# calclavia/tal-asrd

Measured on AMD Instinct MI355X. Metric: audio frames/sec (16 kHz, 10 ms hop) end-to-end log-mel -> TDS encoder -> diarization head, higher is better.
Workload: dtype f32 (dense layers: 3 x f16 MFMA hi/lo split, f32 accumulate)

## Files before the change

tal_asrd_amd/csrc/api.hip:

```cpp
#include <string.h>

#include <atomic>

#include "common.h"

namespace tal {

static thread_local char g_err[512] = "";

void set_error(const char* fmt, ...) {
    va_list ap;
    va_start(ap, fmt);
    vsnprintf(g_err, sizeof(g_err), fmt, ap);
    va_end(ap);
}

static const char* const g_opt_names[OPT_COUNT] = {
    "tds_exact_f32", "tds_fp32_activations", "gconv_fuse_split", "gconv_c1_generic", "head_no_astationary", "gemm_global_loads",
    "gemm_no_splitk4", "gemm_no_glds", "gemm_no_splitk_tail", "gemm_no_w64", "logmel_no_fold", "decode_no_small", "decode_small_rows", "gemm_no_row_split", "gemm_no_n96", "gemm_s64_below", "gconv_short_below", "gconv_no_shift18", "gconv_grid_xyz", "gemm_w64_stagger", "gemm_s64_order", "decode_wide_gemm", "gemm_s64_rows", "decode_persist", "decode_persist_wgs", "logmel_mfma", "gru_unfused", "decode_no_fold", "gconv_c1_fuse", "decode_fold_rows", "gconv_long_tt", "logmel_general"};
static std::atomic<int> g_opt[OPT_COUNT] = {{0}, {0}, {0}, {0}, {0}, {0}, {0}, {0}, {0}, {0}, {0}, {0}, {256}, {0}, {0}, {2}, {4}, {0}, {0}, {0}, {0}, {0}, {0}, {0}, {32}, {0}, {0}, {0}, {0}, {64}, {0}, {0}};
int opt(Option o) { return g_opt[o].load(std::memory_order_relaxed); }

int device_cus() {
    static std::atomic<int> table[64];
    int dev = 0;
    if (hipGetDevice(&dev) != hipSuccess || dev < 0 || dev >= 64) dev = 0;
    int cus = table[dev].load(std::memory_order_relaxed);
    if (!cus) {
        hipDeviceProp_t p;
        if (hipGetDeviceProperties(&p, dev) == hipSuccess) cus = p.multiProcessorCount;
        if (cus <= 0) cus = 256;
        table[dev].store(cus, std::memory_order_relaxed);
    }
    return cus;
}

static const int PROF_MAX = 8192;
static std::atomic<bool> g_prof_on{false};
static std::atomic<int> g_prof_n{0};
static hipEvent_t g_prof_ev[PROF_MAX][2];
static std::atomic<int> g_prof_have[PROF_MAX];
static int g_prof_cls[PROF_MAX];
static double g_prof_work[PROF_MAX];

ProfScope::ProfScope(int cls, double work, hipStream_t stream) : slot(-1), s(stream) {
    if (!g_prof_on.load(std::memory_order_relaxed)) return;
    const int mine = g_prof_n.fetch_add(1, std::memory_order_relaxed);
    if (mine >= PROF_MAX) return;
    g_prof_cls[mine] = -1;
    if (!g_prof_have[mine].load(std::memory_order_acquire)) {
        if (hipEventCreate(&g_prof_ev[mine][0]) != hipSuccess || hipEventCreate(&g_prof_ev[mine][1]) != hipSuccess)
            return;
        g_prof_have[mine].store(1, std::memory_order_release);
    }
    slot = mine;
    g_prof_cls[slot] = cls;
    g_prof_work[slot] = work;
    (void)hipEventRecord(g_prof_ev[slot][0], s);
}
ProfScope::~ProfScope() {
    if (slot >= 0) (void)hipEventRecord(g_prof_ev[slot][1], s);
}

__global__ __launch_bounds__(256) void argmax_rows_kernel(const float* __restrict__ x, int64_t M, int N,
                                                         int32_t* __restrict__ ids) {
    const int lane = threadIdx.x & 63;
    const int64_t row = (int64_t)blockIdx.x * 4 + (threadIdx.x >> 6);
    if (row >= M) return;
    const float* xr = x + row * N;
    float best = -INFINITY;
    int bi = 0x7fffffff;
    for (int i = lane; i < N; i += 64) {
        const float v = xr[i];
// ... 701 lines not shown
```

tal_asrd_amd/csrc/common.h:

```cpp
#pragma once
#include <hip/hip_runtime.h>
#include <stdint.h>
#include <stdio.h>
#include <stdarg.h>
#include <stdlib.h>

#include "../../include/tal_asrd.h"

namespace tal {

void set_error(const char* fmt, ...);

#define TAL_CHECK_ARG(cond, ...)                 \
    do {                                         \
        if (!(cond)) {                           \
            tal::set_error(__VA_ARGS__);         \
            return TAL_EINVAL;                   \
        }                                        \
    } while (0)

#define TAL_CHECK_LAUNCH(what)                                                        \
    do {                                                                              \
        hipError_t e__ = hipGetLastError();                                           \
        if (e__ != hipSuccess) {                                                      \
// ... 35 lines not shown
__device__ __forceinline__ void reset_ticket(unsigned* word) {
    __hip_atomic_store(word, 0u, __ATOMIC_RELAXED, __HIP_MEMORY_SCOPE_AGENT);
}

__device__ __forceinline__ float amax4(float a, const f32x4& v) {
    return fmaxf(fmaxf(a, fmaxf(fabsf(v.x), fabsf(v.y))), fmaxf(fabsf(v.z), fabsf(v.w)));
}
__device__ __forceinline__ void note_range(float amax, int* flag) {
    if (flag && amax > 65504.f) atomicOr(flag, 1);
}

typedef float f32x2p __attribute__((ext_vector_type(2)));
typedef _Float16 f16x2p __attribute__((ext_vector_type(2)));
__device__ __forceinline__ void split_f16x3_pair(float a, float b, f16x2p& hi, f16x2p& lo) {
    const f32x2p x = {a, b};
    hi = __builtin_convertvector(x, f16x2p);
    const f32x2p hf = __builtin_convertvector(hi, f32x2p);
    lo = __builtin_convertvector((x - hf) * 2048.f, f16x2p);
}

enum Option {
    OPT_TDS_EXACT_F32 = 0,
    OPT_TDS_FP32_ACTIVATIONS,
    OPT_GCONV_FUSE_SPLIT,
    OPT_GCONV_C1_GENERIC,
    OPT_HEAD_NO_ASTATIONARY,
    OPT_GEMM_GLOBAL_LOADS,
    OPT_GEMM_NO_SPLITK4,
    OPT_GEMM_NO_GLDS,
    OPT_GEMM_NO_SPLITK_TAIL,
    OPT_GEMM_NO_W64,
    OPT_LOGMEL_NO_FOLD,
    OPT_DECODE_NO_SMALL,
    OPT_DECODE_SMALL_ROWS,
    OPT_GEMM_NO_ROW_SPLIT,
    OPT_GEMM_NO_N96,
    OPT_GEMM_S64_BELOW,
    OPT_GCONV_SHORT_BELOW,
    OPT_GCONV_NO_SHIFT18,
    OPT_GCONV_GRID_XYZ,
    OPT_GEMM_W64_STAGGER,
    OPT_GEMM_S64_ORDER,
    OPT_DECODE_WIDE_GEMM,
    OPT_GEMM_S64_ROWS,
    OPT_DECODE_PERSIST,
    OPT_DECODE_PERSIST_WGS,
    OPT_LOGMEL_MFMA,
    OPT_GRU_UNFUSED,
    OPT_DECODE_NO_FOLD,
    OPT_GCONV_C1_FUSE,
    OPT_DECODE_FOLD_ROWS,
    OPT_GCONV_LONG_TT,
    OPT_LOGMEL_GENERAL,
    OPT_COUNT
};
int opt(Option o);
int device_cus();

__device__ __forceinline__ unsigned xcd_logical_block(unsigned nb, unsigned bid) {
    const unsigned xcd = bid & 7u, q = nb >> 3, r = nb & 7u;
    return (xcd < r ? xcd * (q + 1) : r * (q + 1) + (xcd - r) * q) + (bid >> 3);
}

__device__ __forceinline__ int wave_id() { return __builtin_amdgcn_readfirstlane((int)(threadIdx.x >> 6)); }

enum ProfClass { PROF_GEMM = 0, PROF_GCONV_RES = 1, PROF_GCONV_S2 = 2, PROF_LOGMEL = 3, PROF_OTHER = 4, PROF_NCLASS = 5 };
struct ProfScope {
    int slot;
    hipStream_t s;
    ProfScope(int cls, double work, hipStream_t stream);
    ~ProfScope();
};

struct GemmArgs {
    const float* A;
    const float* W;
    const float* bias;
    const float* res;
    float* Y;
    int64_t M;
    int N, K;
    int64_t lda, ldw, ldy, ldres;
    int nb2;
    int64_t a_s1, a_s2, w_s1, w_s2, y_s1, y_s2, r_s1, r_s2, bias_s2;
    float alpha;
    int scale_cols;
    int tiles_n;
    unsigned tiles_n_magic;
    float* part_val;
    int32_t* part_idx;
    int part_ld;
    int tile_base, split, tail_tiles;
    float* splitk_ws;
    size_t splitk_ws_bytes;
    int f16x3, out_split;
    int res_split;
    int* range_flag;
    int stagger_ticks, stagger_blocks;
    int n_major, tiles_m;
    unsigned tiles_m_magic;
};
int launch_gemm(GemmArgs g, int mode, int nbatch, hipStream_t s);
void launch_gemm_w64(const GemmArgs& g, int mode, bool splitk, dim3 grid, hipStream_t s);
bool gemm_s64_ok(const GemmArgs& g, int mode);
void launch_gemm_s64(GemmArgs g, int mode, hipStream_t s);
int gemm_mode4_partials(int64_t M, int N);
// ... 120 lines not shown
```

tal_asrd_amd/csrc/gconv.hip:

```cpp
#include "common.h"

namespace tal {

constexpr int KS = 21;

template <int CIG, int COG, int STRIDE, int GB, int TT, bool RESID>
__global__ __launch_bounds__(256) void gconv_kernel(const float* __restrict__ x, const float* __restrict__ wp,
                                                   const float* __restrict__ bias, float alpha,
                                                   float* __restrict__ y, int64_t T_in, int64_t T_out, int C_in,
                                                   int C_out) {
    constexpr int PAD = RESID ? KS / 2 : 0;
    constexpr int TIN = (TT - 1) * STRIDE + KS;
    constexpr int TINP = TIN | 1;
    constexpr int WPG = GB >= 4 ? 1 : 4 / GB;
    constexpr int TW = TT / WPG;
    constexpr int R = TW / 64;
    static_assert(TW % 64 == 0 && R >= 1, "time tile per wave must be a multiple of 64");
    constexpr int CH = GB * CIG;
    extern __shared__ __attribute__((aligned(16))) float xs[];

    const int b = blockIdx.z;
    const int g0 = blockIdx.y * GB;
    const int64_t t0 = (int64_t)blockIdx.x * TT;
    const int tid = threadIdx.x;
// ... 337 lines not shown
    }
    return false;
}

template <int P>
__device__ __forceinline__ f16x8 gconv_frag(const _Float16* p, const _Float16* p2) {
    if (P % 8 == 0) return *reinterpret_cast<const f16x8*>(p);
#ifdef GC_MERGED_READS
    if (P % 4 == 0) return *reinterpret_cast<const f16x8a8*>(p);
#endif
    if (P % 4 == 0) {
        typedef _Float16 f16x4a8 __attribute__((ext_vector_type(4), aligned(8)));
        const f16x4a8 a = *reinterpret_cast<const f16x4a8*>(p), b = *reinterpret_cast<const f16x4a8*>(p2);
        return f16x8{a[0], a[1], a[2], a[3], b[0], b[1], b[2], b[3]};
    }
    return *reinterpret_cast<const f16x8u*>(p);
}

#ifdef GC_TIMELINE
__device__ unsigned long long g_gc_timeline[8 * 4 * 4096];
#define GC_STAMP(i)                                                                                   \
    do {                                                                                              \
        if ((threadIdx.x & 63) == 0 && blockIdx.x < 4096)                                             \
            g_gc_timeline[((i) * 4 + (threadIdx.x >> 6)) * 4096 + blockIdx.x] = wall_clock64();       \
    } while (0)
#else
#define GC_STAMP(i)
#endif

#define GC_BLOCK_INDEX(n_tt, n_gb)                                                           \
    int b, g0;                                                                               \
    int64_t t0;                                                                              \
    if (n_tt > 0) {                                                                          \
        const unsigned L = xcd_logical_block(gridDim.x, blockIdx.x);                         \
        const unsigned gbi = L % (unsigned)n_gb, rest = L / (unsigned)n_gb;                  \
        g0 = (int)gbi * GB;                                                                  \
        t0 = (int64_t)(rest % (unsigned)n_tt) * TT;                                          \
        b = (int)(rest / (unsigned)n_tt);                                                    \
    } else {                                                                                 \
        b = blockIdx.z;                                                                      \
        g0 = blockIdx.y * GB;                                                                \
        t0 = (int64_t)blockIdx.x * TT;                                                       \
    }

struct GcC1 {
    const float* mel;
    const float* w1;
    const float* b1;
    const float* mean;
    int64_t T_mel;
    int C_mel;
};

template <int CIG, int COG, int STRIDE, bool RESID, int GB, int TT, int SPLIT, bool XSPLIT = false, bool FROMC1 = false>
__global__ __launch_bounds__(256, GC_LB(CIG, STRIDE)) void gconv_mfma_kernel(const float* __restrict__ x, const _Float16* __restrict__ wfrag,
                                                           const float* __restrict__ bias, float alpha, float* __restrict__ y,
                                                           _Float16* __restrict__ ysplit, int64_t T_in, int64_t T_out, int C_in,
                                                           int C_out, int* __restrict__ range_flag, int n_tt, int n_gb, const GcC1 c1) {
    using LY = GcLayout<CIG, STRIDE>;
    constexpr int NKS = LY::NKS, NK0 = LY::nk(0), MT = (COG + 15) / 16;
    constexpr int P0 = LY::pitch(0), P1 = LY::pitch(1);
    constexpr int PADT = RESID ? KS / 2 : 0;
    constexpr bool STAGED = SPLIT == 2 && GB * MT == 4 && (GB * COG) % 4 == 0 && P0 % 4 == 0 && P0 >= (COG < 16 ? 4 * ((COG + 3) / 4) : 16) &&
                            (MT == 1 || (MT == 2 && ((LY::NSEG == 2 && P1 >= 4) || (LY::NSEG == 1 && P0 >= 4 * ((COG + 3) / 4)))));
    constexpr int TIN = (TT - 1) * STRIDE + KS;
    constexpr int SL0 = LY::slab(0, TT), SL1 = LY::slab(1, TT), GS = SL0 + SL1;
    constexpr int CH = GB * CIG, CH4 = CH / 4;
    constexpr int RPP = 256 / CH4;
    static_assert(CH % 4 == 0 && CIG % 2 == 0 && TT % 64 == 0 && (!RESID || (CIG == COG && STRIDE == 1)), "shape");
    extern __shared__ __attribute__((aligned(16))) _Float16 slab[];
    _Float16* s_hi = slab;
    _Float16* s_lo = slab + GB * GS;

    GC_BLOCK_INDEX(n_tt, n_gb)
    const int tid = threadIdx.x, lane = tid & 63;
    const int w = wave_id();
    const float* xb = x + (int64_t)b * T_in * C_in;
    float* yb = y + (int64_t)b * T_out * C_out;
    GC_STAMP(0);

    if constexpr (FROMC1) {
        static_assert(CIG == 10 && COG == 10 && STRIDE == 1 && RESID && GB == 4 && XSPLIT && SPLIT == 2 && LY::NSEG == 1 && TIN % 4 == 0 && P0 % 2 == 0, "shape");
        constexpr int NR = 2 * (TIN - 1) + KS;
        float* xs = reinterpret_cast<float*>(slab + 2 * GB * GS);
        const float* mb = c1.mel + (int64_t)b * c1.T_mel * c1.C_mel + g0;
        const int64_t m0 = 2 * (t0 - PADT);
        for (int i = tid; i < NR; i += 256) {
            int64_t t = m0 + i;
            t = t < 0 ? 0 : (t < c1.T_mel ? t : c1.T_mel - 1);
            *reinterpret_cast<f32x4*>(xs + i * GB) = *reinterpret_cast<const f32x4*>(mb + t * c1.C_mel);
        }
        __syncthreads();
        float amax = 0.f;
        constexpr int NPAIR = GB * CIG / 2, NPH = 256 / NPAIR;
        if (tid < NPAIR * NPH) {
            typedef float f32x2 __attribute__((ext_vector_type(2)));
            const int pr = tid % NPAIR, ph = tid / NPAIR;
            const int gl = pr / (CIG / 2), ci = 2 * (pr - gl * (CIG / 2)), g = g0 + gl;
            f32x2 wk[KS];
#pragma unroll
            for (int k = 0; k < KS; ++k) wk[k] = *reinterpret_cast<const f32x2*>(c1.w1 + ((int64_t)g * KS + k) * COG + ci);
            f32x2 bv = *reinterpret_cast<const f32x2*>(c1.b1 + g * COG + ci);
            if (c1.mean) {
                f32x2 wsum = wk[0];
#pragma unroll
                for (int k = 1; k < KS; ++k) wsum += wk[k];
                const float m = -c1.mean[0];
                bv[0] = fmaf(m, wsum[0], bv[0]);
// ... 118 lines not shown
                        const f32x2 xc2 = {__builtin_amdgcn_fmed3f(v[u][2 * q], -65504.f, 65504.f),
                                           __builtin_amdgcn_fmed3f(v[u][2 * q + 1], -65504.f, 65504.f)};
                        const f16x2 hh = __builtin_convertvector(xc2, f16x2);
                        const f32x2 hf = __builtin_convertvector(hh, f32x2);
                        const f16x2 ll = __builtin_convertvector((xc2 - hf) * 2048.f, f16x2);
                        *reinterpret_cast<f16x2*>(s_hi + so[q] + tbase + row * sp[q]) = hh;
                        *reinterpret_cast<f16x2*>(s_lo + so[q] + tbase + row * sp[q]) = ll;
                        if constexpr (MAXPAD > 0) pad_row(q, so[q] + tbase + row * sp[q]);
                    }
                }
            }
        }
        note_range(amax, range_flag);
        const f16x2 z2 = {(_Float16)0.f, (_Float16)0.f};
#pragma unroll
        for (int sg = 0; sg < LY::NSEG; ++sg) {
            const int pt = sg ? P1 : P0, rows = LY::rows(sg, TT), sl = sg ? SL1 : SL0, base = sg ? SL0 : 0;
            const int tail2 = (sl - rows * pt) / 2;
            if (tail2 > 0)
                for (int i = tid; i < 2 * GB * tail2; i += 256)
                    *reinterpret_cast<f16x2*>(slab + (i / tail2) * GS + base + rows * pt + 2 * (i % tail2)) = z2;
        }
    }
    GC_STAMP(1);
    __syncthreads();
    GC_STAMP(2);

    constexpr int NU = GB * MT, NB = TT / 16;
    constexpr int UPW = NU >= 4 ? NU / 4 : 1;
    constexpr int WPU = NU >= 4 ? 1 : 4 / NU;
    constexpr int NBW = NB / WPU;
    static_assert(NU == 1 || NU == 2 || NU % 4 == 0, "units");
    const int col = lane & 15, kg = lane >> 4;
    for (int uu = 0; uu < UPW; ++uu) {
        const int u = NU >= 4 ? w + 4 * uu : w / WPU;
        const int part = NU >= 4 ? 0 : w % WPU;
        const int gl = u / MT, mt = u - gl * MT, g = g0 + gl;
        f16x8 wh[NKS], wl[NKS];
        const f16x8* wf = reinterpret_cast<const f16x8*>(wfrag) + (int64_t)(g * MT + mt) * (NKS * 2 * 64) + lane;
#pragma unroll
        for (int ks = 0; ks < NKS; ++ks) {
            wh[ks] = wf[(ks * 2 + 0) * 64];
            wl[ks] = wf[(ks * 2 + 1) * 64];
        }
        const int ch0 = mt * 16 + 4 * kg;
        const int nvalid = COG - ch0;
        f32x4 bv = {0.f, 0.f, 0.f, 0.f};
#pragma unroll
        for (int i = 0; i < 4; ++i)
            if (i < nvalid) bv[i] = bias[g * COG + ch0 + i];
        const int tbeg = part * NBW, tend = (part + 1) * NBW;
        asm volatile("" :: "v"(wh[NKS - 1]), "v"(wl[NKS - 1]));
        GC_STAMP(4);
        constexpr int NKP = LY::NKP;
        const int kgo = LY::PERM ? 64 * (kg & 1) + 32 * (kg >> 1) : 8 * kg;
        const _Float16* hs = s_hi + gl * GS + kgo;
        const _Float16* ls = s_lo + gl * GS + kgo;
        int four = 4;
        asm volatile("" : "+v"(four));
        const _Float16* hs2 = hs + four;
        const _Float16* ls2 = ls + four;
        const _Float16* hst = s_hi + gl * GS + 8 * kg;
        const _Float16* lst = s_lo + gl * GS + 8 * kg;
        const _Float16* hst2 = hst + four;
        const _Float16* lst2 = lst + four;
        int boff0 = (tbeg * 16 + col) * P0, boff1 = SL0 + (tbeg * 16 + col) * P1;
        auto frag_off = [&](int c, int b0, int b1) {
            return c < NKP ? b0 + 128 * (c >> 2) + 8 * (c & 3) : (c < NK0 ? b0 + 32 * c : b1 + 32 * (c - NK0));
        };
        auto frag = [&](const _Float16* base, int c, int b0, int b1) {
            const bool is_hi = base == hs;
            const bool plain = LY::PERM && c >= NKP;
            const _Float16* b1p = plain ? (is_hi ? hst : lst) : base;
            const _Float16* b2p = plain ? (is_hi ? hst2 : lst2) : (is_hi ? hs2 : ls2);
            return c < NK0 ? gconv_frag<P0>(b1p + frag_off(c, b0, b1), b2p + frag_off(c, b0, b1))
                           : gconv_frag<P1>(b1p + frag_off(c, b0, b1), b2p + frag_off(c, b0, b1));
        };
        constexpr int PF = GC_PF, RING = PF + 1;
        static_assert(PF >= 1 && PF < NKS, "prefetch depth");
        f16x8 ch[PF], cl[PF];
#pragma unroll
        for (int q = 0; q < PF; ++q) {
            ch[q] = frag(hs, q, boff0, boff1);
            cl[q] = frag(ls, q, boff0, boff1);
        }
        constexpr int XD = 3;
        static_assert(NBW % (XD + 1) == 0, "blocks per wave");
        const int cbase = g * COG + ch0;
        const float* xcol = xb + cbase + (nvalid >= 4 ? 0 : (nvalid == 2 ? -2 : -ch0));
        auto load_x = [&](int tb) {
            int64_t t = t0 + tb * 16 + col;
            t = t < T_out ? t : T_out - 1;
            return *reinterpret_cast<const f32x4u*>(xcol + t * C_in);
        };
        f32x4 xr[XD + 1];
        if (RESID && !XSPLIT) {
#pragma unroll
            for (int j = 0; j < XD; ++j) xr[j] = load_x(tbeg + j);
        }
        const int rseg = (STRIDE == 1 && LY::NSEG == 2 && ch0 >= LY::nch(0)) ? 1 : 0;
        const _Float16* rh = s_hi + gl * GS + (rseg ? SL0 + ch0 - LY::nch(0) : ch0);
        const _Float16* rl = s_lo + gl * GS + (rseg ? SL0 + ch0 - LY::nch(0) : ch0);
        const int rp = rseg ? P1 : P0;
        constexpr int r01 = 0;
        const int r23 = nvalid >= 4 ? 2 : 0;
        const int rows_left = (int)(T_out - t0 < (int64_t)TT ? T_out - t0 : (int64_t)TT) - col;
// ... 494 lines not shown
    const int i = (int)(idx % S18_WLP), c = (int)((idx / S18_WLP) & 1), g = (int)(idx / (2 * S18_WLP));
    const int k = i - S18_WPRE;
    float v = 0.f;
    if (k >= 0 && k < KS * 20) {
        const int j = k / 20, cc = k - 20 * j;
        if (cc < 18) v = src[((int64_t)(g * 18 + 16 + c) * 18 + cc) * KS + j];
    }
    _Float16 hi, lo;
    split_f16x3(v, hi, lo);
    _Float16* line = dst + ((int64_t)(g * 2 + c) * 2) * S18_WLP + i;
    line[0] = hi;
    line[S18_WLP] = lo;
}

__global__ void pack_gconv_mfma_kernel(const float* __restrict__ src, _Float16* __restrict__ dst, const GcPackDesc d) {
    const int nks = d.nk[0] + d.nk[1];
    const int64_t total = (int64_t)d.groups * d.mt_n * nks * 64 * 8;
    const int64_t idx = (int64_t)blockIdx.x * blockDim.x + threadIdx.x;
    if (idx >= total) return;
    const int i = (int)(idx & 7), l = (int)((idx >> 3) & 63);
    int64_t r = idx >> 9;
    const int c = (int)(r % nks);
    r /= nks;
    const int mt = (int)(r % d.mt_n), g = (int)(r / d.mt_n);
    const int sg = c < d.nk[0] ? 0 : 1, ks = c - (sg ? d.nk[0] : 0);
    const int kg = l >> 4;
    const int co = mt * 16 + (l & 15);
    const int k = (sg == 0 && ks < d.perm_nk) ? 128 * (ks >> 2) + 8 * (ks & 3) + 64 * (kg & 1) + 32 * (kg >> 1) + i : 32 * ks + 8 * kg + i;
    const int j = k / d.pitch[sg], cc = k - j * d.pitch[sg];
    float v = 0.f;
    if (co < d.cog && j < d.ntap[sg] && cc < d.nch[sg])
        v = src[((int64_t)(g * d.cog + co) * d.cig + d.choff[sg] + cc) * KS + d.tap0[sg] + j * d.tapstep];
    _Float16 hi, lo;
    split_f16x3(v, hi, lo);
    const int64_t base = ((((int64_t)(g * d.mt_n + mt) * nks + c) * 2) * 64 + l) * 8 + i;
    dst[base] = hi;
    dst[base + 64 * 8] = lo;
}

template <int CIG, int GB>
static constexpr bool g0_aligned() { return (CIG * GB) % 4 == 0; }

static dim3 gconv_grid(int64_t tiles, int group_blocks, int B, int& n_tt, int& n_gb) {
    const int64_t nb = tiles * group_blocks * B;
    if (nb < (1ll << 31) && tiles < (1ll << 31) && !opt(OPT_GCONV_GRID_XYZ)) {
        n_tt = (int)tiles;
        n_gb = group_blocks;
        return dim3((unsigned)nb);
    }
    n_tt = n_gb = 0;
    return dim3((unsigned)tiles, (unsigned)group_blocks, (unsigned)B);
}

template <int CIG, int COG, int STRIDE, bool RESID, int GB, int TT>
static int launch_mfma_spec(const float* x, const void* wfrag, const float* bias, float alpha, float* y, void* ysplit, int B,
                            int64_t T_in, int64_t T_out, int C_in, int C_out, int groups, hipStream_t s, int* range_flag,
                            bool x_split = false) {
    using LY = GcLayout<CIG, STRIDE>;
    constexpr size_t lds = (size_t)2 * GB * (LY::slab(0, TT) + LY::slab(1, TT)) * sizeof(_Float16);
    typedef void (*kern_t)(const float*, const _Float16*, const float*, float, float*, _Float16*, int64_t, int64_t, int, int, int*, int, int, const GcC1);
    kern_t k;
    if (x_split) k = y ? (ysplit ? (kern_t)gconv_mfma_kernel<CIG, COG, STRIDE, RESID, GB, TT, 1, true> : (kern_t)gconv_mfma_kernel<CIG, COG, STRIDE, RESID, GB, TT, 0, true>)
                       : (kern_t)gconv_mfma_kernel<CIG, COG, STRIDE, RESID, GB, TT, 2, true>;
    else k = y ? (ysplit ? (kern_t)gconv_mfma_kernel<CIG, COG, STRIDE, RESID, GB, TT, 1, false> : (kern_t)gconv_mfma_kernel<CIG, COG, STRIDE, RESID, GB, TT, 0, false>)
               : (kern_t)gconv_mfma_kernel<CIG, COG, STRIDE, RESID, GB, TT, 2, false>;
    TAL_CHECK_ARG(y || ysplit, "gconv (fp16x3): no output buffer");
    TAL_CHECK_ARG(!ysplit || C_out % 32 == 0, "gconv (fp16x3): the split output needs C_out %% 32 == 0");
    TAL_CHECK_ARG(!x_split || (C_in % 32 == 0 && (g0_aligned<CIG, GB>())), "gconv (fp16x3): the split input needs C_in %% 32 == 0");
    static const void* attr_done[6] = {};
    const int slot = (x_split ? 3 : 0) + (y ? (ysplit ? 1 : 0) : 2);
    if (attr_done[slot] != reinterpret_cast<const void*>(k)) {
        if (hipFuncSetAttribute(reinterpret_cast<const void*>(k), hipFuncAttributeMaxDynamicSharedMemorySize, (int)lds) != hipSuccess) {
            set_error("gconv (fp16x3): cannot reserve %zu bytes of LDS", lds);
            return TAL_EHIP;
        }
        attr_done[slot] = reinterpret_cast<const void*>(k);
    }
    int n_tt, n_gb;
    const dim3 grid = gconv_grid(cdiv(T_out, TT), groups / GB, B, n_tt, n_gb);
    ProfScope prof(RESID ? PROF_GCONV_RES : PROF_GCONV_S2, 2.0 * (double)B * (double)T_out * C_out * CIG * KS, s);
    hipLaunchKernelGGL(k, grid, dim3(256), lds, s, x, reinterpret_cast<const _Float16*>(wfrag), bias, alpha, y,
                       reinterpret_cast<_Float16*>(ysplit), T_in, T_out, C_in, C_out, range_flag, n_tt, n_gb, GcC1{});
    TAL_CHECK_LAUNCH("gconv (fp16x3)");
    return TAL_OK;
}

static bool gconv_short_tiles(int64_t T_out, int tt_long, int group_blocks, int B) {
    return cdiv(T_out, tt_long) * group_blocks * B < (int64_t)opt(OPT_GCONV_SHORT_BELOW) * device_cus();
}

bool gconv_f16x3_fits(int64_t T, int C) { return T * C * 4 + (int64_t)300 * C * 4 < ((int64_t)1 << 31); }

static size_t gconv_f16x3_main_halves(const GcPackDesc& d) { return (size_t)d.groups * d.mt_n * (d.nk[0] + d.nk[1]) * 2 * 64 * 8; }
static bool gconv_has_shift18(const GcPackDesc& d) { return d.cig == 18 && d.cog == 18 && d.tapstep == 1 && d.nseg == 1 && d.pitch[0] == 20; }

size_t gconv_f16x3_weight_bytes(int C_in, int C_out, int groups, int stride) {
    if (groups <= 0 || C_in % groups || C_out % groups) return 0;
    GcPackDesc d;
    if (!gconv_mfma_desc(C_in / groups, C_out / groups, stride, groups, d)) return 0;
    return gconv_f16x3_main_halves(d) * sizeof(_Float16) + (gconv_has_shift18(d) ? (size_t)groups * 4 * S18_WLP * sizeof(_Float16) : 0);
}

int launch_pack_gconv_f16x3(const float* w_ref, void* w_frag, int C_in, int C_out, int groups, int stride, hipStream_t s) {
    TAL_CHECK_ARG(w_ref && w_frag, "tal_pack_gconv_f16x3_weight: null pointer");
    GcPackDesc d;
    TAL_CHECK_ARG(groups > 0 && C_in % groups == 0 && C_out % groups == 0 && gconv_mfma_desc(C_in / groups, C_out / groups, stride, groups, d),
                  "tal_pack_gconv_f16x3_weight: no fp16x3 kernel for %d -> %d channels, groups=%d, stride %d", C_in, C_out, groups, stride);
    const int64_t total = (int64_t)groups * d.mt_n * (d.nk[0] + d.nk[1]) * 64 * 8;
    hipLaunchKernelGGL(pack_gconv_mfma_kernel, dim3((unsigned)cdiv(total, 256)), dim3(256), 0, s, w_ref, reinterpret_cast<_Float16*>(w_frag), d);
    TAL_CHECK_LAUNCH("tal_pack_gconv_f16x3_weight");
    if (gconv_has_shift18(d)) {
        const int64_t ts = (int64_t)groups * 2 * S18_WLP;
        hipLaunchKernelGGL(pack_gconv_shift18_kernel, dim3((unsigned)cdiv(ts, 256)), dim3(256), 0, s, w_ref,
                           reinterpret_cast<_Float16*>(w_frag) + gconv_f16x3_main_halves(d), groups);
        TAL_CHECK_LAUNCH("tal_pack_gconv_f16x3_weight (shifted tile)");
// ... 28 lines not shown
    TAL_CHECK_LAUNCH("gconv (resize conv + TDSBlock conv)");
    return TAL_OK;
}
int launch_gconv_c1_res_f16x3(const float* mel, const float* w1, const float* b1, const float* in_mean, const void* w_frag, const float* bias,
                              float alpha, int B, int64_t T_mel, int groups, void* y_split, hipStream_t s, int* range_flag) {
    TAL_CHECK_ARG(mel && w1 && b1 && w_frag && bias && y_split, "gconv (resize conv + TDSBlock conv): null pointer");
    TAL_CHECK_ARG(B > 0 && T_mel >= KS && gconv_c1_res_fusable(groups, 10 * groups, groups, mel), "gconv (resize conv + TDSBlock conv): shape not supported");
    const int64_t T1 = (T_mel - KS) / 2 + 1;
    const int C = 10 * groups;
    TAL_CHECK_ARG(gconv_f16x3_fits(T1, C), "gconv (resize conv + TDSBlock conv): one batch item must stay below 2 GiB");
    GcC1 c1 = {mel, w1, b1, in_mean, T_mel, groups};
    if (gconv_short_tiles(T1, 256, groups / 4, B)) return launch_c1_res_tt<64>(c1, w_frag, bias, alpha, B, T1, C, groups, y_split, s, range_flag);
    return launch_c1_res_tt<256>(c1, w_frag, bias, alpha, B, T1, C, groups, y_split, s, range_flag);
}

int launch_gconv_res_f16x3(const float* x, const void* w_frag, const float* bias, float alpha, int B, int64_t T, int C, int groups,
                           float* y, void* y_split, hipStream_t s, int* range_flag, bool x_split) {
    TAL_CHECK_ARG(x && w_frag && bias && (y || y_split), "tal_gconv_res_f16x3_fwd: null pointer");
    TAL_CHECK_ARG((const void*)x != (const void*)y && (const void*)x != y_split, "tal_gconv_res_f16x3_fwd: in-place not supported (halo reads)");
    TAL_CHECK_ARG(gconv_f16x3_weight_bytes(C, C, groups, 1) > 0, "tal_gconv_res_f16x3_fwd: no fp16x3 kernel for C=%d groups=%d", C, groups);
    TAL_CHECK_ARG(B > 0 && T > 0, "tal_gconv_res_f16x3_fwd: bad shape");
    TAL_CHECK_ARG(!y_split || C % 32 == 0, "tal_gconv_res_f16x3_fwd: the split output needs C %% 32 == 0 (C=%d)", C);
    TAL_CHECK_ARG((reinterpret_cast<uintptr_t>(x) & 15) == 0 && C % 4 == 0, "tal_gconv_res_f16x3_fwd: x must be 16-byte aligned");
    TAL_CHECK_ARG(gconv_f16x3_fits(T, C), "tal_gconv_res_f16x3_fwd: one batch item must stay below 2 GiB (T=%lld, C=%d)", (long long)T, C);
    const int cg = C / groups;
    if (cg == 18 && x_split && !y && y_split && GC_P18 == 20 && GC_KPERM && !opt(OPT_GCONV_NO_SHIFT18)) {
        GcPackDesc d;
        gconv_mfma_desc(18, 18, 1, groups, d);
        const _Float16* wshift = reinterpret_cast<const _Float16*>(w_frag) + gconv_f16x3_main_halves(d);
        const bool shortt = gconv_short_tiles(T, 256, groups / 2, B);
        using LY = GcLayout<18, 1>;
        const size_t lds = ((size_t)2 * 2 * LY::slab(0, shortt ? 64 : 256) + (size_t)2 * 4 * S18_WLP) * sizeof(_Float16);
        auto kern = shortt ? gconv18_shift_kernel<64> : gconv18_shift_kernel<256>;
        static const void* attr_done[2] = {};
        if (attr_done[shortt] != reinterpret_cast<const void*>(kern)) {
            if (hipFuncSetAttribute(reinterpret_cast<const void*>(kern), hipFuncAttributeMaxDynamicSharedMemorySize, (int)lds) != hipSuccess) {
                set_error("gconv (fp16x3, shifted tile): cannot reserve %zu bytes of LDS", lds);
                return TAL_EHIP;
            }
            attr_done[shortt] = reinterpret_cast<const void*>(kern);
        }
        int n_tt, n_gb;
        dim3 grid = gconv_grid(cdiv(T, shortt ? 64 : 256), groups / 2, B, n_tt, n_gb);
        const int nb_total = n_tt > 0 ? (int)grid.x : 0;
#ifdef GC_S18_PERSIST
        if (n_tt > 0 && grid.x > 2u * (unsigned)device_cus()) grid = dim3(2u * (unsigned)device_cus());
#endif
        ProfScope prof(PROF_GCONV_RES, 2.0 * (double)B * (double)T * C * cg * KS, s);
        hipLaunchKernelGGL(kern, grid, dim3(256), lds, s, x, reinterpret_cast<const _Float16*>(w_frag), wshift, bias, alpha,
                           reinterpret_cast<_Float16*>(y_split), T, C, range_flag, n_tt, n_gb, nb_total);
        TAL_CHECK_LAUNCH("gconv (fp16x3, shifted tile)");
        return TAL_OK;
    }
    if (gconv_short_tiles(T, 256, groups / (cg == 18 ? 2 : 4), B)) {
        if (cg == 10) return launch_mfma_spec<10, 10, 1, true, 4, 64>(x, w_frag, bias, alpha, y, y_split, B, T, T, C, C, groups, s, range_flag, x_split);
        if (cg == 14) return launch_mfma_spec<14, 14, 1, true, 4, 64>(x, w_frag, bias, alpha, y, y_split, B, T, T, C, C, groups, s, range_flag, x_split);
        return launch_mfma_spec<18, 18, 1, true, 2, 64>(x, w_frag, bias, alpha, y, y_split, B, T, T, C, C, groups, s, range_flag, x_split);
    }
    const int long_tt = opt(OPT_GCONV_LONG_TT);
    if (long_tt == 128 && cg == 10) return launch_mfma_spec<10, 10, 1, true, 4, 128>(x, w_frag, bias, alpha, y, y_split, B, T, T, C, C, groups, s, range_flag, x_split);
    if (long_tt != 256 && cg == 14) return launch_mfma_spec<14, 14, 1, true, 4, 128>(x, w_frag, bias, alpha, y, y_split, B, T, T, C, C, groups, s, range_flag, x_split);
    if (cg == 10) return launch_mfma_spec<10, 10, 1, true, 4, 256>(x, w_frag, bias, alpha, y, y_split, B, T, T, C, C, groups, s, range_flag, x_split);
    if (cg == 14) return launch_mfma_spec<14, 14, 1, true, 4, 256>(x, w_frag, bias, alpha, y, y_split, B, T, T, C, C, groups, s, range_flag, x_split);
    return launch_mfma_spec<18, 18, 1, true, 2, 256>(x, w_frag, bias, alpha, y, y_split, B, T, T, C, C, groups, s, range_flag, x_split);
}

int launch_gconv_s2_f16x3(const float* x, const void* w_frag, const float* bias, int B, int64_t T_in, int C_in, int C_out, int groups,
                          float* y, hipStream_t s, int* range_flag, bool x_split, void* y_split) {
    TAL_CHECK_ARG(x && w_frag && bias && (y || y_split), "tal_gconv_s2_f16x3_fwd: null pointer");
    TAL_CHECK_ARG(gconv_f16x3_weight_bytes(C_in, C_out, groups, 2) > 0, "tal_gconv_s2_f16x3_fwd: no fp16x3 kernel for %d -> %d channels, groups=%d",
                  C_in, C_out, groups);
    TAL_CHECK_ARG(B > 0 && T_in >= KS, "tal_gconv_s2_f16x3_fwd: T_in=%lld shorter than the kernel", (long long)T_in);
    TAL_CHECK_ARG((reinterpret_cast<uintptr_t>(x) & 15) == 0 && C_in % 4 == 0, "tal_gconv_s2_f16x3_fwd: x must be 16-byte aligned");
    TAL_CHECK_ARG(gconv_f16x3_fits(T_in, C_in), "tal_gconv_s2_f16x3_fwd: one batch item must stay below 2 GiB (T=%lld, C=%d)", (long long)T_in, C_in);
    const int64_t T_out = (T_in - KS) / 2 + 1;
    if (gconv_short_tiles(T_out, 128, groups / (C_in / groups == 10 ? 4 : 2), B)) {
        if (C_in / groups == 10) return launch_mfma_spec<10, 14, 2, false, 4, 64>(x, w_frag, bias, 0.f, y, y_split, B, T_in, T_out, C_in, C_out, groups, s, range_flag, x_split);
        return launch_mfma_spec<14, 18, 2, false, 2, 64>(x, w_frag, bias, 0.f, y, y_split, B, T_in, T_out, C_in, C_out, groups, s, range_flag, x_split);
    }
    if (C_in / groups == 10) return launch_mfma_spec<10, 14, 2, false, 4, 128>(x, w_frag, bias, 0.f, y, y_split, B, T_in, T_out, C_in, C_out, groups, s, range_flag, x_split);
    return launch_mfma_spec<14, 18, 2, false, 2, 128>(x, w_frag, bias, 0.f, y, y_split, B, T_in, T_out, C_in, C_out, groups, s, range_flag, x_split);
}

__global__ void pack_gconv_kernel(const float* __restrict__ src, float* __restrict__ dst, int c_out, int cig, int ks,
                                  int groups) {
    const int total = c_out * cig * ks;
    const int i = blockIdx.x * blockDim.x + threadIdx.x;
    if (i >= total) return;
    const int cog = c_out / groups;
    const int co = i % cog;
    int t = i / cog;
    const int k = t % ks;
    t /= ks;
    const int ci = t % cig;
    const int g = t / cig;
    dst[i] = src[((g * cog + co) * cig + ci) * ks + k];
}

}

#ifdef GC_TIMELINE
extern "C" int tal_debug_gconv_timeline(void* host_out) {
    return hipMemcpyFromSymbol(host_out, HIP_SYMBOL(tal::g_gc_timeline), sizeof(tal::g_gc_timeline)) == hipSuccess ? 0 : -3;
}
#endif

extern "C" int tal_pack_gconv_weight(const float* w_ref, float* w_packed, int c_out, int c_in_per_group, int ksize,
                                     int groups, void* stream) {
    TAL_CHECK_ARG(w_ref && w_packed, "tal_pack_gconv_weight: null pointer");
    TAL_CHECK_ARG(ksize == tal::KS, "tal_pack_gconv_weight: kernel size %d (only 21 is built)", ksize);
    TAL_CHECK_ARG(groups > 0 && c_out % groups == 0 && c_in_per_group > 0, "tal_pack_gconv_weight: bad shape");
    const int total = c_out * c_in_per_group * ksize;
    hipLaunchKernelGGL(tal::pack_gconv_kernel, dim3((total + 255) / 256), dim3(256), 0, (hipStream_t)stream, w_ref,
// ... 5 lines not shown
```

Before: 21.22 million.

## Share input fragments across adjacent output blocks in 14-channel residual gconv

```diff
diff --git a/tal_asrd_amd/csrc/api.hip b/tal_asrd_amd/csrc/api.hip
--- a/tal_asrd_amd/csrc/api.hip
+++ b/tal_asrd_amd/csrc/api.hip
@@ -17,8 +17,8 @@
 
 static const char* const g_opt_names[OPT_COUNT] = {
     "tds_exact_f32", "tds_fp32_activations", "gconv_fuse_split", "gconv_c1_generic", "head_no_astationary", "gemm_global_loads",
-    "gemm_no_splitk4", "gemm_no_glds", "gemm_no_splitk_tail", "gemm_no_w64", "logmel_no_fold", "decode_no_small", "decode_small_rows", "gemm_no_row_split", "gemm_no_n96", "gemm_s64_below", "gconv_short_below", "gconv_no_shift18", "gconv_grid_xyz", "gemm_w64_stagger", "gemm_s64_order", "decode_wide_gemm", "gemm_s64_rows", "decode_persist", "decode_persist_wgs", "logmel_mfma", "gru_unfused", "decode_no_fold", "gconv_c1_fuse", "decode_fold_rows", "gconv_long_tt", "logmel_general"};
-static std::atomic<int> g_opt[OPT_COUNT] = {{0}, {0}, {0}, {0}, {0}, {0}, {0}, {0}, {0}, {0}, {0}, {0}, {256}, {0}, {0}, {2}, {4}, {0}, {0}, {0}, {0}, {0}, {0}, {0}, {32}, {0}, {0}, {0}, {0}, {64}, {0}, {0}};
+    "gemm_no_splitk4", "gemm_no_glds", "gemm_no_splitk_tail", "gemm_no_w64", "logmel_no_fold", "decode_no_small", "decode_small_rows", "gemm_no_row_split", "gemm_no_n96", "gemm_s64_below", "gconv_short_below", "gconv_no_shift18", "gconv_grid_xyz", "gemm_w64_stagger", "gemm_s64_order", "decode_wide_gemm", "gemm_s64_rows", "decode_persist", "decode_persist_wgs", "logmel_mfma", "gru_unfused", "decode_no_fold", "gconv_c1_fuse", "decode_fold_rows", "gconv_long_tt", "logmel_general", "gconv_no_shared_frags"};
+static std::atomic<int> g_opt[OPT_COUNT] = {{0}, {0}, {0}, {0}, {0}, {0}, {0}, {0}, {0}, {0}, {0}, {0}, {256}, {0}, {0}, {2}, {4}, {0}, {0}, {0}, {0}, {0}, {0}, {0}, {32}, {0}, {0}, {0}, {0}, {64}, {0}, {0}, {0}};
 int opt(Option o) { return g_opt[o].load(std::memory_order_relaxed); }
 
 int device_cus() {
diff --git a/tal_asrd_amd/csrc/common.h b/tal_asrd_amd/csrc/common.h
--- a/tal_asrd_amd/csrc/common.h
+++ b/tal_asrd_amd/csrc/common.h
@@ -111,6 +111,7 @@
     OPT_DECODE_FOLD_ROWS,
     OPT_GCONV_LONG_TT,
     OPT_LOGMEL_GENERAL,
+    OPT_GCONV_NO_SHARED_FRAGS,
     OPT_COUNT
 };
 int opt(Option o);
diff --git a/tal_asrd_amd/csrc/gconv.hip b/tal_asrd_amd/csrc/gconv.hip
--- a/tal_asrd_amd/csrc/gconv.hip
+++ b/tal_asrd_amd/csrc/gconv.hip
@@ -413,8 +413,8 @@
     int C_mel;
 };
 
-template <int CIG, int COG, int STRIDE, bool RESID, int GB, int TT, int SPLIT, bool XSPLIT = false, bool FROMC1 = false>
-__global__ __launch_bounds__(256, GC_LB(CIG, STRIDE)) void gconv_mfma_kernel(const float* __restrict__ x, const _Float16* __restrict__ wfrag,
+template <int CIG, int COG, int STRIDE, bool RESID, int GB, int TT, int SPLIT, bool XSPLIT = false, bool FROMC1 = false, int SHF = 1>
+__global__ __launch_bounds__(256, SHF > 1 && TT <= 128 ? 3 : GC_LB(CIG, STRIDE)) void gconv_mfma_kernel(const float* __restrict__ x, const _Float16* __restrict__ wfrag,
                                                            const float* __restrict__ bias, float alpha, float* __restrict__ y,
                                                            _Float16* __restrict__ ysplit, int64_t T_in, int64_t T_out, int C_in,
                                                            int C_out, int* __restrict__ range_flag, int n_tt, int n_gb, const GcC1 c1) {
@@ -639,6 +639,115 @@
         const int tbeg = part * NBW, tend = (part + 1) * NBW;
         asm volatile("" :: "v"(wh[NKS - 1]), "v"(wl[NKS - 1]));
         GC_STAMP(4);
+        if constexpr (SHF > 1) {
+            static_assert(RESID && XSPLIT && STAGED && MT == 1 && LY::NSEG == 1 && !LY::PERM && P0 == 16 && STRIDE == 1 && WPU == 1,
+                          "shared fragments: 14-channel TDSBlock conv, split form in and out");
+            constexpr int SR = 8, SC = SR * P0 / 32, NJ = NK0 + SC * (SHF - 1), SB = 16 * SHF, NSB = TT / SB;
+            static_assert(TT % SB == 0, "super blocks per tile");
+            const int cst = (col & 7) + 8 * SHF * (col >> 3);
+            const _Float16* hsf = s_hi + gl * GS + 8 * kg;
+            const _Float16* lsf = s_lo + gl * GS + 8 * kg;
+            const _Float16* rh = s_hi + gl * GS + ch0;
+            const _Float16* rl = s_lo + gl * GS + ch0;
+            const int r23 = nvalid >= 4 ? 2 : 0;
+            const int nrows = (int)(T_out - t0 < (int64_t)TT ? T_out - t0 : (int64_t)TT);
+            constexpr int PF = 1, RING = PF + 1;
+            static_assert(PF >= 1 && PF < NJ, "prefetch depth");
+            int boff = cst * P0;
+            f16x8 ch[PF], cl[PF];
+#pragma unroll
+            for (int q = 0; q < PF; ++q) {
+                ch[q] = *reinterpret_cast<const f16x8*>(hsf + boff + 32 * q);
+                cl[q] = *reinterpret_cast<const f16x8*>(lsf + boff + 32 * q);
+            }
+            typedef float f32x2 __attribute__((ext_vector_type(2)));
+            typedef _Float16 f16x4a8 __attribute__((ext_vector_type(4), aligned(8)));
+            const f32x2 s11 = {1.0f / 2048.0f, 1.0f / 2048.0f}, z0 = {0.f, 0.f}, al2 = {alpha, alpha};
+            float am = 0.f;
+#pragma unroll 1
+            for (int sb = 0; sb < NSB; ++sb) {
+                f32x4 acc[SHF], ax1[SHF], ax2[SHF];
+#pragma unroll
+                for (int h = 0; h < SHF; ++h) {
+                    acc[h] = bv;
+                    ax1[h] = f32x4{0.f, 0.f, 0.f, 0.f};
+                    ax2[h] = f32x4{0.f, 0.f, 0.f, 0.f};
+                }
+                const int nb = sb + 1 < NSB ? boff + SB * P0 : boff;
+                f16x8 bh[RING], bl[RING];
+#pragma unroll
+                for (int q = 0; q < PF; ++q) {
+                    bh[q] = ch[q];
+                    bl[q] = cl[q];
+                }
+#pragma unroll
+                for (int j = 0; j < NJ; ++j) {
+                    const int pk = j + PF;
+                    const int po = pk < NJ ? boff + 32 * pk : nb + 32 * (pk - NJ);
+                    bh[pk % RING] = *reinterpret_cast<const f16x8*>(hsf + po);
+                    bl[pk % RING] = *reinterpret_cast<const f16x8*>(lsf + po);
+                    __builtin_amdgcn_sched_barrier(0);
+#pragma unroll
+                    for (int h = 0; h < SHF; ++h) {
+                        const int c = j - SC * h;
+                        if (c >= 0 && c < NK0) {
+                            acc[h] = __builtin_amdgcn_mfma_f32_16x16x32_f16(wh[c], bh[j % RING], acc[h], 0, 0, 0);
+                            ax1[h] = __builtin_amdgcn_mfma_f32_16x16x32_f16(wh[c], bl[j % RING], ax1[h], 0, 0, 0);
+                            ax2[h] = __builtin_amdgcn_mfma_f32_16x16x32_f16(wl[c], bh[j % RING], ax2[h], 0, 0, 0);
+                        }
+                    }
+                    __builtin_amdgcn_sched_barrier(0);
+                }
+#pragma unroll
+                for (int q = 0; q < PF; ++q) {
+                    ch[q] = bh[(NJ + q) % RING];
+                    cl[q] = bl[(NJ + q) % RING];
+                }
+                const int sl0 = sb * SB + cst;
+                f16x2 h01[SHF], l01[SHF], h23[SHF], l23[SHF];
+#pragma unroll
+                for (int h = 0; h < SHF; ++h) {
+                    const int ro = (sl0 + 8 * h + PADT) * P0;
+                    h01[h] = *reinterpret_cast<const f16x2*>(rh + ro);
+                    l01[h] = *reinterpret_cast<const f16x2*>(rl + ro);
+                    h23[h] = *reinterpret_cast<const f16x2*>(rh + ro + r23);
+                    l23[h] = *reinterpret_cast<const f16x2*>(rl + ro + r23);
+                }
+#pragma unroll
+                for (int h = 0; h < SHF; ++h) {
+                    f32x2 oa = {acc[h][0], acc[h][1]}, ob = {acc[h][2], acc[h][3]};
+                    {
+                        const f32x2 xa = {ax1[h][0] + ax2[h][0], ax1[h][1] + ax2[h][1]}, xb2 = {ax1[h][2] + ax2[h][2], ax1[h][3] + ax2[h][3]};
+                        oa = xa * s11 + oa;
+                        ob = xb2 * s11 + ob;
+                    }
+                    const f32x2 xa = __builtin_convertvector(l01[h], f32x2) * s11 + __builtin_convertvector(h01[h], f32x2);
+                    const f32x2 xb2 = __builtin_convertvector(l23[h], f32x2) * s11 + __builtin_convertvector(h23[h], f32x2);
+                    oa = al2 * __builtin_elementwise_max(oa, z0) + xa;
+                    ob = al2 * __builtin_elementwise_max(ob, z0) + xb2;
+                    const int sl = sl0 + 8 * h;
+                    float am2 = __builtin_fmaxf(am, __builtin_fmaxf(__builtin_fabsf(oa[0]), __builtin_fabsf(oa[1])));
+                    if (nvalid >= 4) am2 = __builtin_fmaxf(am2, __builtin_fmaxf(__builtin_fabsf(ob[0]), __builtin_fabsf(ob[1])));
+                    am = sl < nrows ? am2 : am;
+                    f16x2p h01p, l01p, h23p, l23p;
+                    if (range_flag) {
+                        split_f16x3_pair(oa[0], oa[1], h01p, l01p);
+                        split_f16x3_pair(ob[0], ob[1], h23p, l23p);
+                    } else {
+                        _Float16 hh[4], ll[4];
+                        split_f16x3(oa[0], hh[0], ll[0]); split_f16x3(oa[1], hh[1], ll[1]);
+                        split_f16x3(ob[0], hh[2], ll[2]); split_f16x3(ob[1], hh[3], ll[3]);
+                        h01p = {hh[0], hh[1]}; l01p = {ll[0], ll[1]}; h23p = {hh[2], hh[3]}; l23p = {ll[2], ll[3]};
+                    }
+                    const int so2 = gl * GS + sl * P0 + 4 * kg;
+                    *reinterpret_cast<f16x4a8*>(s_hi + so2) = f16x4a8{h01p[0], h01p[1], h23p[0], h23p[1]};
+                    *reinterpret_cast<f16x4a8*>(s_lo + so2) = f16x4a8{l01p[0], l01p[1], l23p[0], l23p[1]};
+                }
+                boff = nb;
+            }
+            note_range(am, range_flag);
+            continue;
+        }
         constexpr int NKP = LY::NKP;
         const int kgo = LY::PERM ? 64 * (kg & 1) + 32 * (kg >> 1) : 8 * kg;
         const _Float16* hs = s_hi + gl * GS + kgo;
@@ -1239,7 +1348,7 @@
     return dim3((unsigned)tiles, (unsigned)group_blocks, (unsigned)B);
 }
 
-template <int CIG, int COG, int STRIDE, bool RESID, int GB, int TT>
+template <int CIG, int COG, int STRIDE, bool RESID, int GB, int TT, int SHF = 1>
 static int launch_mfma_spec(const float* x, const void* wfrag, const float* bias, float alpha, float* y, void* ysplit, int B,
                             int64_t T_in, int64_t T_out, int C_in, int C_out, int groups, hipStream_t s, int* range_flag,
                             bool x_split = false) {
@@ -1247,7 +1356,10 @@
     constexpr size_t lds = (size_t)2 * GB * (LY::slab(0, TT) + LY::slab(1, TT)) * sizeof(_Float16);
     typedef void (*kern_t)(const float*, const _Float16*, const float*, float, float*, _Float16*, int64_t, int64_t, int, int, int*, int, int, const GcC1);
     kern_t k;
-    if (x_split) k = y ? (ysplit ? (kern_t)gconv_mfma_kernel<CIG, COG, STRIDE, RESID, GB, TT, 1, true> : (kern_t)gconv_mfma_kernel<CIG, COG, STRIDE, RESID, GB, TT, 0, true>)
+    if constexpr (SHF > 1) {
+        TAL_CHECK_ARG(x_split && !y && ysplit, "gconv (fp16x3, shared fragments): split form in and out only");
+        k = gconv_mfma_kernel<CIG, COG, STRIDE, RESID, GB, TT, 2, true, false, SHF>;
+    } else if (x_split) k = y ? (ysplit ? (kern_t)gconv_mfma_kernel<CIG, COG, STRIDE, RESID, GB, TT, 1, true> : (kern_t)gconv_mfma_kernel<CIG, COG, STRIDE, RESID, GB, TT, 0, true>)
                        : (kern_t)gconv_mfma_kernel<CIG, COG, STRIDE, RESID, GB, TT, 2, true>;
     else k = y ? (ysplit ? (kern_t)gconv_mfma_kernel<CIG, COG, STRIDE, RESID, GB, TT, 1, false> : (kern_t)gconv_mfma_kernel<CIG, COG, STRIDE, RESID, GB, TT, 0, false>)
                : (kern_t)gconv_mfma_kernel<CIG, COG, STRIDE, RESID, GB, TT, 2, false>;
@@ -1382,13 +1494,17 @@
         TAL_CHECK_LAUNCH("gconv (fp16x3, shifted tile)");
         return TAL_OK;
     }
+    const bool shf = cg == 14 && x_split && !y && y_split && !opt(OPT_GCONV_NO_SHARED_FRAGS);
     if (gconv_short_tiles(T, 256, groups / (cg == 18 ? 2 : 4), B)) {
+        if (shf) return launch_mfma_spec<14, 14, 1, true, 4, 64, 2>(x, w_frag, bias, alpha, y, y_split, B, T, T, C, C, groups, s, range_flag, x_split);
         if (cg == 10) return launch_mfma_spec<10, 10, 1, true, 4, 64>(x, w_frag, bias, alpha, y, y_split, B, T, T, C, C, groups, s, range_flag, x_split);
         if (cg == 14) return launch_mfma_spec<14, 14, 1, true, 4, 64>(x, w_frag, bias, alpha, y, y_split, B, T, T, C, C, groups, s, range_flag, x_split);
         return launch_mfma_spec<18, 18, 1, true, 2, 64>(x, w_frag, bias, alpha, y, y_split, B, T, T, C, C, groups, s, range_flag, x_split);
     }
     const int long_tt = opt(OPT_GCONV_LONG_TT);
     if (long_tt == 128 && cg == 10) return launch_mfma_spec<10, 10, 1, true, 4, 128>(x, w_frag, bias, alpha, y, y_split, B, T, T, C, C, groups, s, range_flag, x_split);
+    if (shf && long_tt != 256) return launch_mfma_spec<14, 14, 1, true, 4, 128, 2>(x, w_frag, bias, alpha, y, y_split, B, T, T, C, C, groups, s, range_flag, x_split);
+    if (shf) return launch_mfma_spec<14, 14, 1, true, 4, 256, 2>(x, w_frag, bias, alpha, y, y_split, B, T, T, C, C, groups, s, range_flag, x_split);
     if (long_tt != 256 && cg == 14) return launch_mfma_spec<14, 14, 1, true, 4, 128>(x, w_frag, bias, alpha, y, y_split, B, T, T, C, C, groups, s, range_flag, x_split);
     if (cg == 10) return launch_mfma_spec<10, 10, 1, true, 4, 256>(x, w_frag, bias, alpha, y, y_split, B, T, T, C, C, groups, s, range_flag, x_split);
     if (cg == 14) return launch_mfma_spec<14, 14, 1, true, 4, 256>(x, w_frag, bias, alpha, y, y_split, B, T, T, C, C, groups, s, range_flag, x_split);
```

Result: no change. 21.23 million, median of 6 (+0.1%).
